# unitaryfoundation/qrack

Hardware: NVIDIA H100
Metric: gates/sec at 30q random circuit; Apply2x2 HBM GB/s vs roofline (higher is better)
Workload: dtype f32

## Files before the change

### qrack_b200/csrc/fused.cu

```cuda
#include "sv_common.cuh"

#include <algorithm>
#include <atomic>
#include <cstdio>
#include <cstdlib>
#include <cstring>
#include <memory>
#include <mutex>

namespace b200sv {

constexpr int FUSED_KC = 12;
constexpr int FUSED_NT = 256;
constexpr int FUSED_RB = 4;
constexpr int FUSED_MINB = 2;
constexpr int FUSED_L = 6;

constexpr int MAX_HIGH = 8;
constexpr int MAX_PASS = 8;
constexpr int MAX_OPS = 96;
constexpr int MAX_HOST_OPS = 384;
constexpr int MAX_SLOTS = 128;
constexpr int MAX_NCH = 16;
constexpr int MAX_NA = 32;
constexpr int MAX_JR = 6;

enum { K_XSWAP = 0, K_GEN_U = 1, K_GEN_P = 2 };
constexpr uint32_t OPC_PHGEN = 15U;
constexpr uint32_t OPC_SCALE = 16U;
constexpr uint32_t OPC_STAGE = 17U;
constexpr uint32_t OPC_PH2 = 18U;
constexpr int ST_SM_SHIFT = 6, ST_ANY_BIT = 12, ST_ACT_SHIFT = 13, ST_RM_SHIFT = 19, ST_CNT_BITS = 4;
constexpr uint32_t ST_MASK = 63U, ST_CNT_MASK = 15U;
constexpr uint32_t CODE_HAS_SB = 0x100U;
constexpr uint32_t CODE_HAS_OUTER = 0x200U;
constexpr int MAX_MEMBERS = 320;
enum { OP_GENERAL = 0, OP_HAD = 1, OP_XSWAP = 2, OP_PHASE = 3, OP_ROT = 4 };

template <typename R> struct alignas(16) DevOp {
    uint64_t omask, oval;
    uint32_t code;
    uint32_t emask;
    uint32_t lmaskSb;
    uint32_t lvalSb;
    R m[8];
};
struct DevPass {
    int opBegin, opEnd;
    int nsb;
    int nIt;
    unsigned char sbit[16];
    unsigned short pswzB[MAX_NCH];
    unsigned short itoffC[16];
    unsigned int pad;
    uint64_t goff[MAX_NCH];
};

struct alignas(16) DevSweep {
    int nHigh;
    int lowAmpBits;
    int kc;
    int nPass;
    int nOps;
    int hasScale;
    double scale;
    int nOuter;
    int outerOff;
    int reserved;
    int nSlots;
    int scratchBytes;
    int directIn;
    int directOut;
    int nMem;
    int memOff;
    int nRot;
    int rotOff;
    int needFull;
    unsigned short slotBeg[MAX_SLOTS + 1];
    uint64_t highLow[MAX_HIGH];
    uint64_t highPow[MAX_HIGH];
    DevPass pass[MAX_PASS];
};

__device__ __forceinline__ uint4 ld_stream(const uint4* p)
{
    uint4 v;
    asm volatile("ld.global.cs.v4.u32 {%0,%1,%2,%3}, [%4];" : "=r"(v.x), "=r"(v.y), "=r"(v.z), "=r"(v.w) : "l"(p));
    return v;
}
__device__ __forceinline__ void st_stream(uint4* p, const uint4 v)
{
    asm volatile("st.global.cs.v4.u32 [%0], {%1,%2,%3,%4};" ::"l"(p), "r"(v.x), "r"(v.y), "r"(v.z), "r"(v.w) : "memory");
}

__host__ __device__ __forceinline__ uint32_t swz(uint32_t c) { return c ^ ((c >> 3) & 7U) ^ ((c >> 6) & 7U) ^ ((c >> 9) & 7U); }

typedef unsigned long long ull;
__device__ __forceinline__ ull pk(float lo, float hi)
{
    ull r;
    asm("mov.b64 %0, {%1,%2};" : "=l"(r) : "f"(lo), "f"(hi));
    return r;
}
__device__ __forceinline__ ull swp64(ull v)
{
    float lo, hi;
    asm("mov.b64 {%0,%1}, %2;" : "=f"(lo), "=f"(hi) : "l"(v));
    return pk(hi, lo);
}
__device__ __forceinline__ float2 upk(ull v)
{
    float2 f;
    asm("mov.b64 {%0,%1}, %2;" : "=f"(f.x), "=f"(f.y) : "l"(v));
    return f;
}
__device__ __forceinline__ ull f2add(ull a, ull b)
{
    const float2 x = upk(a), y = upk(b);
    return pk(__fadd_rn(x.x, y.x), __fadd_rn(x.y, y.y));
}
__device__ __forceinline__ ull f2mul(ull a, ull b)
{
    const float2 x = upk(a), y = upk(b);
    return pk(__fmul_rn(x.x, y.x), __fmul_rn(x.y, y.y));
}
__device__ __forceinline__ ull f2fma(ull a, ull b, ull c)
{
    const float2 x = upk(a), y = upk(b), z = upk(c);
    return pk(__fmaf_rn(x.x, y.x, z.x), __fmaf_rn(x.y, y.y, z.y));
}

template <typename R> struct AmpOps;
template <> struct AmpOps<float> {
    typedef ull A;
    typedef ulonglong2 Chunk;
    static constexpr int APC = 2;
    struct Ph {
        ull xx, ny;
    };
    static __device__ __forceinline__ Ph mkph(float x, float y) { return Ph{ pk(x, x), pk(-y, y) }; }
    static __device__ __forceinline__ A mulc(A a, const Ph& p) { return f2fma(a, p.xx, f2mul(swp64(a), p.ny)); }
    static __device__ __forceinline__ A macc(A a, const Ph& p, A acc) { return f2fma(a, p.xx, f2fma(swp64(a), p.ny, acc)); }
    static __device__ __forceinline__ void had(A& x, A& y)
    {
        x = f2add(x, y);
        y = f2fma(y, pk(-2.0f, -2.0f), x);
    }
    static __device__ __forceinline__ void rot(A& x, A& y, float c, float s)
    {
        const ull cc = pk(c, c), ss = pk(s, s), ns = pk(-s, -s);
        const A nx = f2fma(x, cc, f2mul(y, ns));
        y = f2fma(y, cc, f2mul(x, ss));
        x = nx;
    }
    static __device__ __forceinline__ A scale(A a, float s) { return f2mul(a, pk(s, s)); }
    static __device__ __forceinline__ A unit() { return pk(1.0f, 0.0f); }
    static __device__ __forceinline__ Ph toph(A a)
    {
        float x, y;
        asm("mov.b64 {%0,%1}, %2;" : "=f"(x), "=f"(y) : "l"(a));
        return mkph(x, y);
    }
    static __device__ __forceinline__ void get(const Chunk& c, A* a)
    {
        a[0] = c.x;
        a[1] = c.y;
    }
    static __device__ __forceinline__ Chunk put(const A* a)
    {
        Chunk c;
        c.x = a[0];
// ... 826 lines not shown
        } else {
            h.kind = OP_GENERAL;
        }
        push(h);
    };
    static const double HS = 0.70710678118654752440;
    static const double HM[8] = { HS, 0, HS, 0, HS, 0, -HS, 0 };
    static const double XM[8] = { 0, 0, 1, 0, 1, 0, 0, 0 };
    uint64_t xpend = 0;
    auto emit_bare_x = [&](int q) {
        if (hist[q].empty() || out[(size_t)hist[q].back()].kind != OP_HAD || out[(size_t)hist[q].back()].tq != q) {
            emit_u1(q, XM);
        } else {
            emit_u1(q, HM);
            emit_phase1(q, 1, -1.0, 0.0);
            emit_u1(q, HM);
        }
    };
    for (const HostOp& op0 : ops) {
        HostOp op = op0;
        op.cval ^= (op.cmask & xpend);
        if (op.kind == OP_XSWAP && !op.cmask) {
            xpend ^= bitq(op.tq);
            continue;
        }
        if (op.tq >= 0 && (xpend & bitq(op.tq))) {
            xpend &= ~bitq(op.tq);
            if (is_u1(op) && op.kind == OP_HAD) {
                emit_u1(op.tq, op.m);
                emit_phase1(op.tq, 1, -1.0, 0.0);
                continue;
            }
            if (is_u1(op)) {
                double mx[8] = { op.m[2], op.m[3], op.m[0], op.m[1], op.m[6], op.m[7], op.m[4], op.m[5] };
                emit_u1(op.tq, mx);
                continue;
            }
            emit_bare_x(op.tq);
        }
        if (op.kind == OP_XSWAP) {
            emit_u1(op.tq, HM);
            HostOp z;
            memset(&z, 0, sizeof(z));
            z.kind = OP_PHASE;
            z.tq = -1;
            z.cmask = op.cmask | bitq(op.tq);
            z.cval = op.cval | bitq(op.tq);
            z.m[0] = -1.0;
            push(z);
            emit_u1(op.tq, HM);
        } else if (is_u1(op)) {
            emit_u1(op.tq, op.m);
        } else if (op.kind == OP_PHASE && op.cmask && !(op.cmask & (op.cmask - 1U))) {
            emit_phase1(__builtin_ctzll(op.cmask), op.cval ? 1 : 0, op.m[0], op.m[1]);
        } else if (op.kind == OP_PHASE && !op.cmask) {
            const double nx = gx * op.m[0] - gy * op.m[1];
            gy = gx * op.m[1] + gy * op.m[0];
            gx = nx;
        } else {
            push(op);
        }
    }
    uint64_t xtail = 0;
    if (__builtin_popcountll(xpend) > 4) {
        xtail = xpend;
    } else {
        for (uint64_t m = xpend; m; m &= m - 1U) {
            emit_bare_x(__builtin_ctzll(m));
        }
    }
    std::vector<HostOp> res;
    res.reserve(out.size() + 1);
    for (size_t i = 0; i < out.size(); ++i) {
        if (!alive[i]) {
            continue;
        }
        const HostOp& h = out[i];
        if (h.kind == OP_GENERAL && !h.cmask) {
            const double* m = h.m;
            const double n00 = m[0] * m[0] + m[1] * m[1], n10 = m[4] * m[4] + m[5] * m[5];
            const double n01 = m[2] * m[2] + m[3] * m[3], n11 = m[6] * m[6] + m[7] * m[7];
            const double ox = m[0] * m[2] + m[1] * m[3] + m[4] * m[6] + m[5] * m[7], oy = m[0] * m[3] - m[1] * m[2] + m[4] * m[7] - m[5] * m[6];
            if (fabs(n00 + n10 - 1.0) < 1e-5 && fabs(n01 + n11 - 1.0) < 1e-5 && fabs(ox) < 1e-5 && fabs(oy) < 1e-5 && n10 > 1e-24 && n01 > 1e-24) {
                const double c = sqrt(n00), sn = sqrt(n10);
                double g0x = 1.0, g0y = 0.0;
                if (c > 1e-12) {
                    g0x = m[0] / c;
                    g0y = m[1] / c;
                }
                const double s01 = sqrt(n01);
                const double ax = (m[4] * g0x + m[5] * g0y) / sn, ay = (m[5] * g0x - m[4] * g0y) / sn;
                const double bx = -(m[2] * g0x + m[3] * g0y) / s01, by = -(m[3] * g0x - m[2] * g0y) / s01;
                const double sm = 0.5 * (sn + s01);
                const double nx = gx * g0x - gy * g0y;
                gy = gx * g0y + gy * g0x;
                gx = nx;
                HostOp ph;
                memset(&ph, 0, sizeof(ph));
                ph.kind = OP_PHASE;
                ph.tq = -1;
                ph.cmask = bitq(h.tq);
                ph.cval = bitq(h.tq);
                if (bx != 1.0 || by != 0.0) {
                    ph.m[0] = bx;
                    ph.m[1] = by;
                    res.push_back(ph);
                }
                HostOp r;
                memset(&r, 0, sizeof(r));
                r.kind = OP_ROT;
                r.tq = h.tq;
                r.m[0] = c;
                r.m[1] = sm;
                res.push_back(r);
                if (ax != 1.0 || ay != 0.0) {
                    ph.m[0] = ax;
                    ph.m[1] = ay;
                    res.push_back(ph);
                }
                continue;
            }
        }
        res.push_back(h);
    }
    if (gx != 1.0 || gy != 0.0) {
        HostOp h;
        memset(&h, 0, sizeof(h));
        h.kind = OP_PHASE;
        h.tq = -1;
        h.m[0] = gx;
        h.m[1] = gy;
        res.push_back(h);
    }
    ops.swap(res);
    return xtail;
}

struct TileCfg {
    int n;
    int apcLog;
    int L;
    int kA;
    int H;
    int maxOps;
};

static TileCfg make_cfg(int n, int prec)
{
    TileCfg c;
    c.n = n;
    c.apcLog = (prec == 32) ? 1 : 0;
    const int kAmax = FUSED_KC + c.apcLog;
    c.kA = std::min(n, kAmax);
    c.L = std::min(FUSED_L, c.kA);
    if (n <= kAmax) {
        c.L = c.kA;
    }
    c.H = c.kA - c.L;
    c.maxOps = MAX_HOST_OPS;
    return c;
}

template <typename FitFn, typename FreeFn>
static void greedy_select(std::vector<HostOp>& pending, std::vector<HostOp>& taken, size_t maxTake, size_t lookahead, FitFn fits,
    FreeFn isFree)
{
    uint64_t blockedT = 0, blockedD = 0;
    std::vector<char> gone(pending.size(), 0);
    std::vector<size_t> deferred;
    uint64_t deferredQ = 0;
    bool nonDiagLeft = false;
    size_t i = 0;
    for (; i < pending.size(); ++i) {
        const HostOp& op = pending[i];
        if (i >= lookahead || taken.size() >= maxTake) {
            break;
        }
        const uint64_t usesT = op.tq >= 0 ? bitq(op.tq) : 0;
        const uint64_t usesD = op.cmask;
        bool conflict = (usesT & (blockedT | blockedD)) || (usesD & blockedT);
        if (!conflict && op.kind == OP_PHASE && !isFree(op)) {
            deferred.push_back(i);
            deferredQ |= usesD;
            continue;
        }
        if (!conflict && !fits(op)) {
            conflict = true;
        }
        if (conflict) {
            blockedT |= usesT;
            blockedD |= usesD;
            nonDiagLeft = nonDiagLeft || op.kind != OP_PHASE;
        } else {
            if (usesT & deferredQ) {
                size_t w = 0;
                deferredQ = 0;
                for (size_t k = 0; k < deferred.size(); ++k) {
                    const size_t j = deferred[k];
                    if ((pending[j].cmask & usesT) && taken.size() + 1U < maxTake) {
                        taken.push_back(pending[j]);
                        gone[j] = 1;
                    } else {
                        deferred[w++] = j;
                        deferredQ |= pending[j].cmask;
                    }
                }
                deferred.resize(w);
                if (usesT & deferredQ) {
                    blockedT |= usesT;
                    blockedD |= usesD;
                    nonDiagLeft = true;
                    continue;
                }
            }
            taken.push_back(op);
            gone[i] = 1;
        }
    }
    for (size_t k = i; k < pending.size() && !nonDiagLeft; ++k) {
        nonDiagLeft = pending[k].kind != OP_PHASE;
    }
    if (!nonDiagLeft) {
        for (size_t k = 0; k < pending.size() && taken.size() < maxTake; ++k) {
            if (!gone[k]) {
                taken.push_back(pending[k]);
                gone[k] = 1;
            }
        }
    }
    std::vector<HostOp> rest;
    rest.reserve(pending.size());
    for (size_t k = 0; k < pending.size(); ++k) {
        if (!gone[k]) {
            rest.push_back(pending[k]);
        }
    }
    pending.swap(rest);
}

struct PassPlan {
    std::vector<HostOp> ops;
    std::vector<int> regQ;
};
struct SweepPlan {
    std::vector<int> highQ;
    std::vector<PassPlan> passes;
    size_t nOps = 0;
};


static size_t greedy_count(const std::vector<HostOp>& pending, size_t maxTake, size_t lookahead, uint64_t inTile)
{
    uint64_t blockedT = 0, blockedD = 0;
    size_t taken = 0;
    const size_t lim = std::min(pending.size(), lookahead);
    for (size_t i = 0; i < lim && taken < maxTake; ++i) {
        const HostOp& op = pending[i];
        const uint64_t usesT = op.tq >= 0 ? bitq(op.tq) : 0;
        const uint64_t usesD = op.cmask;
        if ((usesT & (blockedT | blockedD)) || (usesD & blockedT) || (usesT & ~inTile)) {
            blockedT |= usesT;
            blockedD |= usesD;
            if (!(inTile & ~(blockedT | blockedD))) {
                break;
            }
        } else {
            ++taken;
        }
    }
    return taken;
}

constexpr int SEARCH_ROUNDS = 2;

static void plan_sweep(std::vector<HostOp>& pending, const TileCfg& cfg, SweepPlan& sp)
{
    uint64_t inTile = (cfg.L >= 64) ? ~0ULL : (bitq(cfg.L) - 1U);
    int freeHigh = cfg.H;
    std::vector<HostOp> sel;
    if (cfg.H > 0 && cfg.n > cfg.L + cfg.H) {
        const uint64_t lowMask = inTile;
        uint64_t cur = lowMask;
        {
            int fh = cfg.H;
            uint64_t bT = 0, bD = 0;
            for (size_t i = 0; i < pending.size() && i < 2048 && fh > 0; ++i) {
                const HostOp& op = pending[i];
                const uint64_t uT = op.tq >= 0 ? bitq(op.tq) : 0, uD = op.cmask;
                if ((uT & (bT | bD)) || (uD & bT)) {
                    bT |= uT;
                    bD |= uD;
                } else if (uT & ~cur) {
                    cur |= uT;
                    --fh;
                }
            }
            for (int q = cfg.n - 1; q >= cfg.L && fh > 0; --q) {
                if (!(cur & bitq(q))) {
                    cur |= bitq(q);
                    --fh;
                }
            }
        }
        size_t best = greedy_count(pending, (size_t)cfg.maxOps, 2048, cur);
        for (int round = 0; round < SEARCH_ROUNDS; ++round) {
            uint64_t bestSet = cur;
            for (int h = cfg.L; h < cfg.n; ++h) {
                if (!(cur & bitq(h))) {
                    continue;
                }
                for (int c = cfg.L; c < cfg.n; ++c) {
                    if (cur & bitq(c)) {
                        continue;
                    }
                    const uint64_t cand = (cur & ~bitq(h)) | bitq(c);
                    const size_t got = greedy_count(pending, (size_t)cfg.maxOps, 2048, cand);
                    if (got > best) {
                        best = got;
                        bestSet = cand;
                    }
                }
            }
            if (bestSet == cur) {
                break;
            }
            cur = bestSet;
        }
        inTile = cur;
        freeHigh = 0;
    }
    greedy_select(
        pending, sel, (size_t)cfg.maxOps, 2048,
        [&](const HostOp& op) {
            if (op.tq < 0 || (inTile & bitq(op.tq))) {
                return true;
            }
            if (freeHigh > 0) {
                inTile |= bitq(op.tq);
                --freeHigh;
                return true;
            }
            return false;
        },
        [&](const HostOp& op) { return freeHigh == 0 && !(op.cmask & inTile); });
    sp.highQ.clear();
    for (int q = cfg.L; q < cfg.n; ++q) {
        if (inTile & bitq(q)) {
            sp.highQ.push_back(q);
        }
    }
    for (int q = cfg.n - 1; q >= cfg.L && (int)sp.highQ.size() < cfg.H; --q) {
        if (!(inTile & bitq(q))) {
            inTile |= bitq(q);
            sp.highQ.push_back(q);
        }
    }
    std::sort(sp.highQ.begin(), sp.highQ.end());
    sp.passes.clear();
    sp.nOps = sel.size();
    while (!sel.empty() && (int)sp.passes.size() < MAX_PASS) {
        PassPlan pp;
        uint64_t regSet = cfg.apcLog ? 1ULL : 0ULL;
        int freeReg = FUSED_RB;
        const uint64_t fixed = regSet;
        uint64_t cur = fixed;
        int fr = FUSED_RB;
        uint64_t bT = 0, bD = 0;
        for (size_t i = 0; i < sel.size() && fr > 0; ++i) {
            const HostOp& op = sel[i];
            const uint64_t uT = op.tq >= 0 ? bitq(op.tq) : 0, uD = op.cmask;
            if ((uT & (bT | bD)) || (uD & bT)) {
                bT |= uT;
                bD |= uD;
            } else if (uT & ~cur) {
                cur |= uT;
                --fr;
            }
        }
        if (fr == 0) {
            size_t best = greedy_count(sel, (size_t)cfg.maxOps, 4096, cur);
            for (int round = 0; round < SEARCH_ROUNDS; ++round) {
                uint64_t bestSet = cur;
                for (uint64_t hm = cur & ~fixed; hm; hm &= hm - 1U) {
                    const uint64_t hbit = hm & (~hm + 1U);
                    for (uint64_t cm = inTile & ~cur; cm; cm &= cm - 1U) {
                        const uint64_t cbit = cm & (~cm + 1U);
                        const uint64_t cand = (cur & ~hbit) | cbit;
                        const size_t got = greedy_count(sel, (size_t)cfg.maxOps, 4096, cand);
                        if (got > best) {
                            best = got;
                            bestSet = cand;
                        }
                    }
                }
                if (bestSet == cur) {
                    break;
                }
                cur = bestSet;
            }
            regSet = cur;
            freeReg = 0;
            for (uint64_t m = cur & ~fixed; m; m &= m - 1U) {
                pp.regQ.push_back(__builtin_ctzll(m));
            }
        }
        greedy_select(
            sel, pp.ops, (size_t)cfg.maxOps, 4096,
            [&](const HostOp& op) {
                if (op.tq < 0 || (regSet & bitq(op.tq))) {
                    return true;
                }
                if (freeReg > 0) {
                    regSet |= bitq(op.tq);
                    --freeReg;
                    pp.regQ.push_back(op.tq);
                    return true;
                }
                return false;
            },
            [&](const HostOp& op) { return !(op.cmask & inTile); });
        sp.passes.push_back(pp);
    }
    if (!sel.empty()) {
        sp.nOps -= sel.size();
        sel.insert(sel.end(), pending.begin(), pending.end());
        pending.swap(sel);
    }
}

static int tile_bit(const TileCfg& cfg, const std::vector<int>& highQ, int q)
{
    if (q < cfg.L) {
        return q;
    }
    for (size_t h = 0; h < highQ.size(); ++h) {
        if (highQ[h] == q) {
            return cfg.L + (int)h;
        }
    }
    return -1;
}

constexpr size_t MAX_PROG_BYTES_2CTA = 24576;

template <typename R>
static size_t encode_sweep(const SweepPlan& sp, const TileCfg& cfg, std::vector<unsigned char>& buf, size_t* scratchOut)
{
    const int kc = cfg.kA - cfg.apcLog;
    const int APC = 1 << cfg.apcLog;
    const int NCH = 1 << FUSED_RB;
    const int NA = NCH * APC;
    int JRN = 0;
    while ((1 << JRN) < NA) {
        ++JRN;
    }
    DevSweep ds;
    memset(&ds, 0, sizeof(ds));
    std::vector<DevOp<R>> dops;
    std::vector<DevOuterPhase<R>> outerList;
    std::vector<std::vector<DevOuterPhase<R>>> slotMembers;
    std::vector<DevMember<R>> memberList;
    std::vector<R> rotList;
    ds.nHigh = (int)sp.highQ.size();
    ds.lowAmpBits = cfg.L;
    ds.kc = kc;
    ds.nPass = (int)sp.passes.size();
    uint64_t tileMask = bitq(cfg.L) - 1U;
    for (int h = 0; h < ds.nHigh; ++h) {
        ds.highLow[h] = bitq(sp.highQ[h]) - 1U;
        ds.highPow[h] = bitq(sp.highQ[h]);
        tileMask |= bitq(sp.highQ[h]);
    }
    double scale = 1.0;
    for (int p = 0; p < ds.nPass; ++p) {
        const PassPlan& pp = sp.passes[p];
        DevPass& dp = ds.pass[p];
        std::vector<int> rb;
        uint32_t used = 0;
        for (int q : pp.regQ) {
            const int cb = tile_bit(cfg, sp.highQ, q) - cfg.apcLog;
            rb.push_back(cb);
            used |= 1U << cb;
        }
        for (int cb = kc - 1; cb >= 0 && (int)rb.size() < FUSED_RB; --cb) {
            if (!(used & (1U << cb))) {
                rb.push_back(cb);
                used |= 1U << cb;
            }
        }
        std::sort(rb.begin(), rb.end());
        std::vector<int> sb;
        uint32_t taken = used;
        for (int pcl = 0; pcl < 3; ++pcl) {
            for (int cand : { pcl, pcl + 3, pcl + 6, pcl + 9 }) {
                if (cand < kc && !(taken & (1U << cand))) {
                    sb.push_back(cand);
                    taken |= 1U << cand;
                    break;
                }
            }
        }
        for (int cb = 0; cb < kc; ++cb) {
            if (!(taken & (1U << cb))) {
                sb.push_back(cb);
                taken |= 1U << cb;
            }
        }
        dp.nsb = (int)sb.size();
        for (size_t i = 0; i < sb.size(); ++i) {
            dp.sbit[i] = (unsigned char)sb[i];
        }
        const uint32_t nSub = 1U << dp.nsb;
        dp.nIt = (int)std::max<uint32_t>(1U, nSub / (uint32_t)FUSED_NT);
        int tidBits = 0;
        while ((1 << tidBits) < FUSED_NT) {
            ++tidBits;
        }
        for (int it = 0; it < dp.nIt && it < 16; ++it) {
            uint32_t off = 0;
            for (int i = tidBits; i < dp.nsb; ++i) {
                if ((it >> (i - tidBits)) & 1) {
                    off |= 1U << sb[i];
                }
            }
            dp.itoffC[it] = (unsigned short)off;
        }
        uint32_t roffA[MAX_NA];
        uint32_t regAmpMask = cfg.apcLog ? 1U : 0U;
        for (int cb : rb) {
            regAmpMask |= 1U << (cb + cfg.apcLog);
        }
        for (int e = 0; e < NCH; ++e) {
            uint32_t off = 0;
            for (int b = 0; b < FUSED_RB; ++b) {
                if ((e >> b) & 1) {
                    off |= 1U << rb[b];
                }
            }
            dp.pswzB[e] = (unsigned short)(swz(off) << 4);
            {
                uint64_t g = 0;
                for (uint32_t ab = off << cfg.apcLog; ab; ab &= ab - 1U) {
                    const int tb = __builtin_ctz(ab);
                    g |= (tb < cfg.L) ? bitq(tb) : bitq(sp.highQ[tb - cfg.L]);
                }
                dp.goff[e] = g;
            }
            for (int w = 0; w < APC; ++w) {
                roffA[e * APC + w] = (off << cfg.apcLog) | (uint32_t)w;
            }
        }
        const uint32_t fullE = (uint32_t)((1ULL << NA) - 1ULL);
        auto reg_index = [&](int tb) {
            int jr = 0;
            for (int b = 0; b < tb; ++b) {
                if (regAmpMask & (1U << b)) {
                    ++jr;
                }
            }
            return jr;
        };
        auto local_pred = [&](const HostOp& hop, uint32_t& lmask, uint32_t& lval) {
            lmask = 0;
            lval = 0;
            for (uint64_t m = hop.cmask & tileMask; m; m &= m - 1U) {
                const int q = __builtin_ctzll(m);
                const int tb = tile_bit(cfg, sp.highQ, q);
                lmask |= 1U << tb;
                if (hop.cval & bitq(q)) {
                    lval |= 1U << tb;
                }
            }
        };
        struct Stage {
            bool h[MAX_JR];
            bool isRot[MAX_JR];
            double rc[MAX_JR], rs[MAX_JR];
            std::vector<DevOuterPhase<R>> slot[MAX_JR];
            std::vector<DevMember<R>> thr[MAX_JR + 1];
            bool any;
        } st;
        auto stage_reset = [&]() {
            for (int b = 0; b < MAX_JR; ++b) {
                st.h[b] = false;
                st.isRot[b] = false;
                st.slot[b].clear();
            }
            for (int g = 0; g < MAX_JR + 1; ++g) {
                st.thr[g].clear();
            }
            st.any = false;
        };
        stage_reset();
        auto stage_slots = [&]() {
            int n = 0;
            for (int b = 0; b < MAX_JR; ++b) {
// ... 141 lines not shown
            for (int e = 0; e < NA; ++e) {
                if ((roffA[e] & lmr) == lvr) {
                    em |= 1U << e;
                }
            }
            d.emask = em;
            const bool uncond = (em == fullE && d.lmaskSb == 0);
            for (int k = 0; k < 8; ++k) {
                d.m[k] = (R)hop.m[k];
            }
            uint32_t code = 0;
            if (hop.kind == OP_PHASE) {
                if (nreg == 2 && lvr == lmr) {
                    const int j = reg_index(__builtin_ctz(lmr)), k = reg_index(31 - __builtin_clz(lmr));
                    code = OPC_PH2 + (uint32_t)(k * (k - 1) / 2 + j);
                } else {
                    code = OPC_PHGEN;
                }
            } else {
                const uint32_t jr = (uint32_t)reg_index(tile_bit(cfg, sp.highQ, hop.tq));
                if (hop.kind == OP_XSWAP) {
                    code = K_XSWAP * 5U + jr;
                } else {
                    code = (uncond ? K_GEN_U : K_GEN_P) * 5U + jr;
                }
            }
            d.code = code | (d.lmaskSb ? CODE_HAS_SB : 0U) | (d.omask ? CODE_HAS_OUTER : 0U);
            if (code < OPC_PHGEN) {
                ds.needFull = 1;
            }
            dops.push_back(d);
        }
        close_stage();
        if (p == ds.nPass - 1 && (scale != 1.0 || !outerList.empty())) {
            DevOp<R> d;
            memset(&d, 0, sizeof(d));
            d.code = OPC_SCALE;
            dops.push_back(d);
        }
        dp.opEnd = (int)dops.size();
    }
    {
        auto lowRegBits = [&](const PassPlan& pp) {
            int cnt = 0;
            for (int q : pp.regQ) {
                const int cb = tile_bit(cfg, sp.highQ, q) - cfg.apcLog;
                if (cb >= 0 && cb < 3) {
                    ++cnt;
                }
            }
            return cnt;
        };
        ds.directIn = (lowRegBits(sp.passes.front()) <= 1) ? 1 : 0;
        ds.directOut = (lowRegBits(sp.passes.back()) <= 1) ? 1 : 0;
    }
    ds.scale = scale;
    if (getenv("B200SV_FUSED_DEBUG")) {
        static const char* names[] = { "XSWAP", "GEN_U", "GEN_P" };
        for (int p = 0; p < ds.nPass; ++p) {
            fprintf(stderr, "  pass %d:", p);
            for (int o = ds.pass[p].opBegin; o < ds.pass[p].opEnd; ++o) {
                const uint32_t c = dops[o].code & 0xffU;
                const char* sfx = (dops[o].code & CODE_HAS_SB) ? "s" : "";
                const char* ofx = dops[o].omask ? "o" : "";
                if (c == OPC_STAGE) {
                    uint32_t cnts = 0;
                    memcpy(&cnts, dops[o].m, sizeof(cnts));
                    int nm = 0, nsl = 0;
                    for (int g = 0; g < MAX_JR + 1; ++g) {
                        nm += (int)((cnts >> (ST_CNT_BITS * g)) & ST_CNT_MASK);
                    }
                    for (int b = 0, sl = (int)dops[o].lmaskSb - 1; b < MAX_JR; ++b) {
                        if ((dops[o].emask >> ST_SM_SHIFT) & (1U << b)) {
                            nsl += (int)slotMembers[sl++].size();
                        }
                    }
                    fprintf(stderr, " STAGE(h%x,s%x:%d,t%d)", dops[o].emask & ST_MASK, (dops[o].emask >> ST_SM_SHIFT) & ST_MASK, nsl, nm);
                } else if (c == OPC_SCALE) {
                    fprintf(stderr, " SCALE");
                } else if (c == OPC_PHGEN) {
                    fprintf(stderr, " PHGEN%s%s", sfx, ofx);
                } else if (c >= OPC_PH2) {
                    fprintf(stderr, " PH2.%u%s%s", c - OPC_PH2, sfx, ofx);
                } else {
                    fprintf(stderr, " %s.%u%s%s", names[c / 5U], c % 5U, sfx, ofx);
                }
            }
            fprintf(stderr, "\n");
        }
        fprintf(stderr, "  sweep: %d ops, %d outer phases, %d thread members, directIn %d, directOut %d\n", (int)dops.size(),
            (int)outerList.size(), (int)memberList.size(), ds.directIn, ds.directOut);
    }
    ds.hasScale = (scale != 1.0 || !outerList.empty()) ? 1 : 0;
    ds.nOps = (int)dops.size();
    ds.nOuter = (int)outerList.size();
    ds.nSlots = 1 + (int)slotMembers.size();
    {
        const int lcb = cfg.L - cfg.apcLog;
        const size_t rows = (size_t)1 << (kc > lcb ? kc - lcb : 0);
        ds.scratchBytes =
            (int)((rows * 8U + (size_t)4 * (size_t)ds.nSlots * sizeof(R) + (size_t)16 * memberList.size() +
                      (size_t)2 * (size_t)ds.nPass * (size_t)FUSED_NT + 15U) & ~(size_t)15U);
    }
    ds.nMem = (int)memberList.size();
    ds.slotBeg[0] = 0;
    ds.slotBeg[1] = (unsigned short)outerList.size();
    for (size_t k = 0; k < slotMembers.size(); ++k) {
        outerList.insert(outerList.end(), slotMembers[k].begin(), slotMembers[k].end());
        ds.slotBeg[k + 2] = (unsigned short)outerList.size();
    }
    const size_t opsBytes = ((dops.size() * sizeof(DevOp<R>)) + 15U) & ~(size_t)15U;
    const size_t outerBytes = ((outerList.size() * sizeof(DevOuterPhase<R>)) + 15U) & ~(size_t)15U;
    const size_t memBytes = memberList.size() * sizeof(DevMember<R>);
    ds.outerOff = (int)(sizeof(DevSweep) + opsBytes);
    ds.memOff = (int)(sizeof(DevSweep) + opsBytes + outerBytes);
    const size_t rotBytes = (rotList.size() * sizeof(R) + 15U) & ~(size_t)15U;
    ds.rotOff = (int)(sizeof(DevSweep) + opsBytes + outerBytes + memBytes);
    ds.nRot = (int)(rotList.size() / 2U);
    const size_t start = buf.size();
    size_t bytes = ((sizeof(DevSweep) + opsBytes + outerBytes + memBytes + rotBytes) + 15U) & ~(size_t)15U;
    if (scratchOut) {
        *scratchOut = (size_t)ds.scratchBytes;
    }
    if (dops.size() > (size_t)MAX_OPS || outerList.size() > 60000U) {
        bytes = (size_t)1 << 30;
        return bytes;
    }
    buf.resize(start + bytes, 0);
    memcpy(buf.data() + start, &ds, sizeof(ds));
    if (!dops.empty()) {
        memcpy(buf.data() + start + sizeof(DevSweep), dops.data(), dops.size() * sizeof(DevOp<R>));
    }
    if (!outerList.empty()) {
        memcpy(buf.data() + start + ds.outerOff, outerList.data(), outerList.size() * sizeof(DevOuterPhase<R>));
    }
    if (!memberList.empty()) {
        memcpy(buf.data() + start + ds.memOff, memberList.data(), memBytes);
    }
    if (!rotList.empty()) {
        memcpy(buf.data() + start + ds.rotOff, rotList.data(), rotList.size() * sizeof(R));
    }
    return bytes;
}

constexpr size_t PLAN_WINDOW = 1024;
static int plan_and_encode(std::vector<HostOp>& pending, const TileCfg& cfg0, int prec, std::vector<unsigned char>& buf, size_t* bytesOut,
    size_t* scratchOut, size_t* nOpsOut, int* nPassOut)
{
    const size_t wsz = std::min(pending.size(), PLAN_WINDOW);
    TileCfg cfg = cfg0;
    for (;;) {
        std::vector<HostOp> window(pending.begin(), pending.begin() + wsz);
        SweepPlan sp;
        plan_sweep(window, cfg, sp);
        if (!sp.nOps) {
            set_error("fused scheduler made no progress");
            return B200SV_ESTATE;
        }
        const size_t mark = buf.size();
        size_t scratch = 0;
        const size_t bytes =
            (prec == 32) ? encode_sweep<float>(sp, cfg, buf, &scratch) : encode_sweep<double>(sp, cfg, buf, &scratch);
        if (bytes + scratch > MAX_PROG_BYTES_2CTA) {
            if (cfg.maxOps <= 4) {
                set_error("fused sweep program does not fit");
                return B200SV_ESTATE;
            }
            buf.resize(mark);
            cfg.maxOps = cfg.maxOps * 3 / 4;
            continue;
        }
        window.insert(window.end(), pending.begin() + wsz, pending.end());
        pending.swap(window);
        *bytesOut = bytes;
        *scratchOut = scratch;
        *nOpsOut = sp.nOps;
        *nPassOut = (int)sp.passes.size();
        return B200SV_OK;
    }
}

struct Seg {
    size_t off, bytes, scratch, nops;
    int npass;
};

static int plan_list(std::vector<HostOp>& pending, const TileCfg& cfg, int prec, std::vector<unsigned char>& buf, std::vector<Seg>& segs)
{
    while (!pending.empty()) {
        const size_t off = buf.size();
        size_t bytes = 0, scratch = 0, nops = 0;
        int npass = 0;
        SV_TRY(plan_and_encode(pending, cfg, prec, buf, &bytes, &scratch, &nops, &npass));
        segs.push_back({ off, bytes, scratch, nops, npass });
        if (getenv("B200SV_FUSED_DEBUG")) {
            fprintf(stderr, "  program %zu B + scratch %zu B\n", bytes, scratch);
        }
    }
    return B200SV_OK;
}

struct Arena {
    unsigned char* dev = nullptr;
    unsigned char* host = nullptr;
    size_t cap = 0;
    cudaEvent_t done = nullptr;
    bool pending = false;
};
static std::vector<std::pair<State*, std::unique_ptr<Arena>>>& arenas()
{
    static std::vector<std::pair<State*, std::unique_ptr<Arena>>> a;
    return a;
}
static std::mutex& arena_mutex()
{
    static std::mutex m;
    return m;
}
static Arena* get_arena(State* s)
{
    std::lock_guard<std::mutex> lk(arena_mutex());
    for (auto& kv : arenas()) {
        if (kv.first == s) {
            return kv.second.get();
        }
    }
    arenas().emplace_back(s, std::unique_ptr<Arena>(new Arena()));
    return arenas().back().second.get();
}
void fused_release(State* s)
{
    std::unique_ptr<Arena> mine;
    {
        std::lock_guard<std::mutex> lk(arena_mutex());
        auto& v = arenas();
        for (size_t i = 0; i < v.size(); ++i) {
            if (v[i].first == s) {
                mine = std::move(v[i].second);
                v.erase(v.begin() + i);
                break;
            }
        }
    }
    if (mine) {
        if (mine->dev) {
            cudaFree(mine->dev);
        }
        if (mine->host) {
            cudaFreeHost(mine->host);
        }
        if (mine->done) {
            cudaEventDestroy(mine->done);
        }
    }
}

bool fused_accepts(const State* s, const GateOp&) { return s->nq >= 5 && s->nq <= 62; }

template <typename R, int VAR, bool PULL = false>
static int launch_sweep_v(State* s, const unsigned char* dprog, uint32_t progBytes, uint32_t scratchBytes, uint64_t nTiles)
{
    auto kern = k_fused_sweep<R, VAR, PULL>;
    const size_t shm = ((size_t)16 << FUSED_KC) + progBytes + scratchBytes;
    static std::atomic<unsigned long long> attr_set_mask{ 0 };
    if (!(attr_set_mask.load() & (1ULL << s->dev))) {
        SV_CUDA(cudaFuncSetAttribute(kern, cudaFuncAttributeMaxDynamicSharedMemorySize, (int)(((size_t)16 << FUSED_KC) + MAX_PROG_BYTES_2CTA)));
        attr_set_mask.fetch_or(1ULL << s->dev);
    }
    const uint64_t maxGrid = (uint64_t)sm_count(s->dev) * FUSED_MINB;
    const unsigned grid = (unsigned)std::min<uint64_t>(nTiles, maxGrid);
    kern<<<grid, FUSED_NT, shm, s->stream>>>(reinterpret_cast<typename Cx<R>::type*>(s->amps), dprog, progBytes, nTiles,
        PULL ? s->pull : PullArgs{});
    SV_CUDA(cudaGetLastError());
    if (PULL) {
        s->amps = s->pull.out;
        s->pullPending = false;
    }
    return B200SV_OK;
}

template <typename R>
static int launch_sweep(State* s, const unsigned char* dprog, uint32_t progBytes, uint32_t scratchBytes, uint64_t nTiles, int var)
{
    return var == 2 ? launch_sweep_v<R, 2>(s, dprog, progBytes, scratchBytes, nTiles)
                    : (var == 1 ? launch_sweep_v<R, 1>(s, dprog, progBytes, scratchBytes, nTiles)
                                : launch_sweep_v<R, 0>(s, dprog, progBytes, scratchBytes, nTiles));
}

int fused_flush(State* s)
{
    if (s->queue.empty()) {
        return s->pullPending ? launch_pull_gather(s) : B200SV_OK;
    }
    if (!s->amps) {
        s->queue.clear();
        return B200SV_OK;
    }
    std::vector<HostOp> pending;
    const uint64_t xtail = lower_queue(s->queue, pending);
    const size_t nGates = s->queue.size();
    const TileCfg cfg = make_cfg(s->nq, s->prec);
    std::vector<unsigned char> buf;
    std::vector<Seg> segs;
    SV_TRY(plan_list(pending, cfg, s->prec, buf, segs));
    s->queue.clear();
    if (s->pullPending && segs.empty()) {
        SV_TRY(launch_pull_gather(s));
// ... 239 lines not shown
        uint64_t base = t << sw.lowAmpBits;
        for (int h = 0; h < sw.nHigh; ++h) {
            const uint64_t lo = base & sw.highLow[h];
            base = ((base ^ lo) << 1) | lo;
        }
        EmuC<R>* const tilePsi = psi + base;
        std::vector<bool> act((size_t)std::max(1, sw.nOps));
        for (int o = 0; o < sw.nOps; ++o) {
            act[o] = (base & ops[o].omask) == ops[o].oval;
        }
        {
            double fx = 1.0, fy = 0.0;
            for (int i = 0; i < sw.nOuter; ++i) {
                if ((base & outer[i].omask) == outer[i].oval) {
                    const double nx = fx * (double)outer[i].ph[0] - fy * (double)outer[i].ph[1];
                    fy = fx * (double)outer[i].ph[1] + fy * (double)outer[i].ph[0];
                    fx = nx;
                }
            }
            tab[0] = (R)(fx * sw.scale);
            tab[1] = (R)(fy * sw.scale);
        }
        for (int sl = 1; sl < sw.nSlots; ++sl) {
            double fx = 1.0, fy = 0.0;
            for (int i = sw.slotBeg[sl]; i < sw.slotBeg[sl + 1]; ++i) {
                if ((base & outer[i].omask) == outer[i].oval) {
                    const double nx = fx * (double)outer[i].ph[0] - fy * (double)outer[i].ph[1];
                    fy = fx * (double)outer[i].ph[1] + fy * (double)outer[i].ph[0];
                    fx = nx;
                }
            }
            tab[2 * sl] = (R)fx;
            tab[2 * sl + 1] = (R)fy;
        }
        for (int i = 0; i < sw.nMem; ++i) {
            const bool ok = (base & members[i].omask) == members[i].oval;
            eff[(size_t)i] = ok ? make_uint2(members[i].lmask, members[i].lval) : make_uint2(0U, 1U);
        }
        if (!sw.directIn) {
            for (uint32_t c = 0; c < nChunk; ++c) {
                for (int w = 0; w < APC; ++w) {
                    const uint64_t off = rowOff[c >> lcb] + (uint64_t)(c & colMask) * APC + w;
                    tile[(size_t)swz(c) * APC + w] = pull ? emu_pull_load<R>(*pull, base + off) : tilePsi[off];
                }
            }
        }
        for (int p = 0; p < sw.nPass; ++p) {
            const DevPass& ps = sw.pass[p];
            const bool fromGlobal = (p == 0) && sw.directIn, toGlobal = (p == sw.nPass - 1) && sw.directOut;
            for (int tid = 0; tid < NT; ++tid) {
                uint32_t dep = 0;
                const int nb = ps.nsb < 8 ? ps.nsb : 8;
                for (int i = 0; i < nb; ++i) {
                    dep |= (((uint32_t)tid >> i) & 1U) << ps.sbit[i];
                }
                for (int it = 0; it < ps.nIt; ++it) {
                    if ((uint32_t)(it * NT + tid) >= nSub) {
                        break;
                    }
                    const uint32_t sbc = dep | ps.itoffC[it];
                    const uint32_t swb = swz(sbc) << 4;
                    EmuC<R>* const gsub = tilePsi + rowOff[sbc >> lcb] + (uint64_t)(sbc & colMask) * APC;
                    for (int e = 0; e < NCH; ++e) {
                        for (int w = 0; w < APC; ++w) {
                            a[(size_t)e * APC + w] = !fromGlobal
                                ? tile[(size_t)((swb ^ ps.pswzB[e]) >> 4) * APC + w]
                                : (pull ? emu_pull_load<R>(*pull, (uint64_t)(gsub - psi) + ps.goff[e] + w) : gsub[ps.goff[e] + w]);
                        }
                    }
                    const uint32_t xsb = sbc * (uint32_t)APC;
                    for (int o = ps.opBegin; o < ps.opEnd; ++o) {
                        if (act[o]) {
                            emu_exec_op<R>(a, ops[o], xsb, tab.data(), NA, members, eff.data(), rotTab);
                        }
                    }
                    for (int e = 0; e < NCH; ++e) {
                        for (int w = 0; w < APC; ++w) {
                            if (toGlobal) {
                                gsub[ps.goff[e] + w] = a[(size_t)e * APC + w];
                            } else {
                                tile[(size_t)((swb ^ ps.pswzB[e]) >> 4) * APC + w] = a[(size_t)e * APC + w];
                            }
                        }
                    }
                }
            }
        }
        if (!sw.directOut) {
            for (uint32_t c = 0; c < nChunk; ++c) {
                for (int w = 0; w < APC; ++w) {
                    tilePsi[rowOff[c >> lcb] + (uint64_t)(c & colMask) * APC + w] = tile[(size_t)swz(c) * APC + w];
                }
            }
        }
    }
}

int fused_emulate(int n_qubits, int precision, const std::vector<GateOp>& q, void* host_state, const PullArgs* pull)
{
    std::vector<HostOp> pending;
    const uint64_t xtail = lower_queue(q, pending);
    const TileCfg cfg = make_cfg(n_qubits, precision);
    std::vector<unsigned char> buf;
    std::vector<Seg> segs;
    SV_TRY(plan_list(pending, cfg, precision, buf, segs));
    if (pull && segs.empty()) {
        const uint64_t dim = 1ULL << n_qubits;
        for (uint64_t i = 0; i < dim; ++i) {
            if (precision == 32) {
                reinterpret_cast<EmuC<float>*>(host_state)[i] = emu_pull_load<float>(*pull, i);
            } else {
                reinterpret_cast<EmuC<double>*>(host_state)[i] = emu_pull_load<double>(*pull, i);
            }
        }
        pull = nullptr;
    }
    for (const Seg& sg : segs) {
        if (precision == 32) {
            emulate_sweep<float>(buf.data() + sg.off, reinterpret_cast<EmuC<float>*>(host_state), n_qubits, cfg, pull);
        } else {
            emulate_sweep<double>(buf.data() + sg.off, reinterpret_cast<EmuC<double>*>(host_state), n_qubits, cfg, pull);
        }
        pull = nullptr;
    }
    if (xtail) {
        const uint64_t dim = 1ULL << n_qubits;
        const size_t ab = (precision == 32) ? 8 : 16;
        unsigned char* st = reinterpret_cast<unsigned char*>(host_state);
        unsigned char tmp[16];
        for (uint64_t i = 0; i < dim; ++i) {
            const uint64_t j = i ^ xtail;
            if (i < j) {
                memcpy(tmp, st + i * ab, ab);
                memcpy(st + i * ab, st + j * ab, ab);
                memcpy(st + j * ab, tmp, ab);
            }
        }
    }
    return B200SV_OK;
}

int fused_plan_gates(int n_qubits, int precision, const std::vector<GateOp>& q, int* n_sweeps, int* n_passes, int* n_ops)
{
    std::vector<HostOp> pending;
    (void)lower_queue(q, pending);
    const TileCfg cfg = make_cfg(n_qubits, precision);
    int sweeps = 0, passes = 0, ops = 0;
    std::vector<unsigned char> buf;
    while (!pending.empty()) {
        size_t bytes = 0, nops = 0, scratch = 0;
        int npass = 0;
        buf.clear();
        SV_TRY(plan_and_encode(pending, cfg, precision, buf, &bytes, &scratch, &nops, &npass));
        ++sweeps;
        passes += npass;
        ops += (int)nops;
    }
    *n_sweeps = sweeps;
    *n_passes = passes;
    *n_ops = ops;
    return B200SV_OK;
}

}
```

Baseline: 5571.

## Shrink low-qubit tile width, fill high slots from low end, defer thin passes

Splits the fixed low-qubit tile width into per-precision values (4 for f32, 3 for f64), which gives more high-qubit slots per sweep, and enlarges the program buffer to match. The default high-qubit fill now picks qubits from the lowest index upward instead of from the top. A final pass with three or fewer ops is pushed back to the next sweep when more work remains. Each of these is meant to cut the number of full-state sweeps over HBM. In exchange, shared-memory use grows and the scattered high strides may make tile loads less coalesced.

```diff
diff --git a/qrack_b200/csrc/fused.cu b/qrack_b200/csrc/fused.cu
--- a/qrack_b200/csrc/fused.cu
+++ b/qrack_b200/csrc/fused.cu
@@ -14,9 +14,10 @@
 constexpr int FUSED_NT = 256;
 constexpr int FUSED_RB = 4;
 constexpr int FUSED_MINB = 2;
-constexpr int FUSED_L = 6;
-
-constexpr int MAX_HIGH = 8;
+constexpr int FUSED_L32 = 4;
+constexpr int FUSED_L64 = 3;
+
+constexpr int MAX_HIGH = (FUSED_KC + 1 - FUSED_L32) > (FUSED_KC - FUSED_L64) ? (FUSED_KC + 1 - FUSED_L32) : (FUSED_KC - FUSED_L64);
 constexpr int MAX_PASS = 8;
 constexpr int MAX_OPS = 96;
 constexpr int MAX_HOST_OPS = 384;
@@ -1149,7 +1150,7 @@
     c.apcLog = (prec == 32) ? 1 : 0;
     const int kAmax = FUSED_KC + c.apcLog;
     c.kA = std::min(n, kAmax);
-    c.L = std::min(FUSED_L, c.kA);
+    c.L = std::min(prec == 32 ? FUSED_L32 : FUSED_L64, c.kA);
     if (n <= kAmax) {
         c.L = c.kA;
     }
@@ -1269,8 +1270,9 @@
 }
 
 constexpr int SEARCH_ROUNDS = 2;
-
-static void plan_sweep(std::vector<HostOp>& pending, const TileCfg& cfg, SweepPlan& sp)
+constexpr int THIN_PASS_OPS = 3;
+
+static void plan_sweep(std::vector<HostOp>& pending, const TileCfg& cfg, SweepPlan& sp, bool more)
 {
     uint64_t inTile = (cfg.L >= 64) ? ~0ULL : (bitq(cfg.L) - 1U);
     int freeHigh = cfg.H;
@@ -1292,7 +1294,7 @@
                     --fh;
                 }
             }
-            for (int q = cfg.n - 1; q >= cfg.L && fh > 0; --q) {
+            for (int q = cfg.L; q < cfg.n && fh > 0; ++q) {
                 if (!(cur & bitq(q))) {
                     cur |= bitq(q);
                     --fh;
@@ -1346,7 +1348,7 @@
             sp.highQ.push_back(q);
         }
     }
-    for (int q = cfg.n - 1; q >= cfg.L && (int)sp.highQ.size() < cfg.H; --q) {
+    for (int q = cfg.L; q < cfg.n && (int)sp.highQ.size() < cfg.H; ++q) {
         if (!(inTile & bitq(q))) {
             inTile |= bitq(q);
             sp.highQ.push_back(q);
@@ -1418,6 +1420,13 @@
             [&](const HostOp& op) { return !(op.cmask & inTile); });
         sp.passes.push_back(pp);
     }
+    if (sp.passes.size() > 1 && sp.passes.back().ops.size() <= (size_t)THIN_PASS_OPS && (more || !pending.empty())) {
+        std::vector<HostOp> back;
+        back.swap(sp.passes.back().ops);
+        sp.passes.pop_back();
+        back.insert(back.end(), sel.begin(), sel.end());
+        sel.swap(back);
+    }
     if (!sel.empty()) {
         sp.nOps -= sel.size();
         sel.insert(sel.end(), pending.begin(), pending.end());
@@ -1438,7 +1447,9 @@
     return -1;
 }
 
-constexpr size_t MAX_PROG_BYTES_2CTA = 24576;
+constexpr size_t MAX_PROG_BYTES_2CTA = 24576 + ((size_t)8 << MAX_HIGH);
+static_assert(FUSED_MINB * (((size_t)16 << FUSED_KC) + MAX_PROG_BYTES_2CTA + 1024 + 1024) <= 228 * 1024,
+    "two fused-sweep CTAs (tile + program + scratch + static shared memory) must fit one SM");
 
 template <typename R>
 static size_t encode_sweep(const SweepPlan& sp, const TileCfg& cfg, std::vector<unsigned char>& buf, size_t* scratchOut)
@@ -1886,7 +1897,7 @@
     for (;;) {
         std::vector<HostOp> window(pending.begin(), pending.begin() + wsz);
         SweepPlan sp;
-        plan_sweep(window, cfg, sp);
+        plan_sweep(window, cfg, sp, pending.size() > wsz);
         if (!sp.nOps) {
             set_error("fused scheduler made no progress");
             return B200SV_ESTATE;
@@ -2432,9 +2443,11 @@
         int npass = 0;
         buf.clear();
         SV_TRY(plan_and_encode(pending, cfg, precision, buf, &bytes, &scratch, &nops, &npass));
+        DevSweep ds;
+        memcpy(&ds, buf.data(), sizeof(ds));
         ++sweeps;
         passes += npass;
-        ops += (int)nops;
+        ops += ds.nOps;
     }
     *n_sweeps = sweeps;
     *n_passes = passes;
```

Result: faster. 5721, median of 6 (+2.7%).
